# linnanwang/FastGen

Measured on AMD Instinct MI355X. Metric: images/sec at 4-step distilled (DMD2) sampling, higher is better.
Workload: dtype fp32 (tensors, accumulate) with split-bf16 x3 MFMA conv products; 1 GPU; EDM CIFAR-10 32x32 SongUNet (55.7M params) DMD2 4-step 'sde' sampling, batch=512 per GPU; global_batch=512, sample_steps=4, parallelism=replicas x1 (no data-path collective), graph=True

## Files before the change

### fastgen_amd/csrc/common.h

```cpp
#pragma once
#include <hip/hip_runtime.h>
#include <stdint.h>

typedef __attribute__((ext_vector_type(8))) __bf16 bf16x8;
typedef __attribute__((ext_vector_type(4))) __bf16 bf16x4;
typedef __attribute__((ext_vector_type(16))) float f32x16;
typedef __attribute__((ext_vector_type(4))) float f32x4;
typedef __attribute__((ext_vector_type(2))) float f32x2;

#define FG_WAVE 64

inline int fg_device_slot() {
    int dev = -1;
    return (hipGetDevice(&dev) == hipSuccess && dev >= 0 && dev < 16) ? dev : -1;
}

template <typename T>
struct DT;
template <>
struct DT<__bf16> {
    typedef __bf16 ST;
    typedef __bf16 WT;
    static constexpr int KC = 64;
    static constexpr int WPARTS = 1;
    static constexpr int FRAG_BYTES = 16;
    static constexpr bool FAST = true;
};
template <>
struct DT<float> {
    typedef float ST;
    typedef float WT;
    static constexpr int KC = 32;
    static constexpr int WPARTS = 1;
    static constexpr int FRAG_BYTES = 32;
    static constexpr bool FAST = false;
};
struct bf16x3 {};
template <>
struct DT<bf16x3> {
    typedef float ST;
    typedef __bf16 WT;
    static constexpr int KC = 32;
    static constexpr int WPARTS = 2;
    static constexpr int FRAG_BYTES = 16;
    static constexpr bool FAST = true;
};

template <typename T>
struct Frag8;
template <>
struct Frag8<__bf16> {
    bf16x8 v;
};
template <>
struct Frag8<float> {
    f32x4 lo, hi;
};
template <>
struct Frag8<bf16x3> {
    bf16x8 hi, lo;
};

__device__ __forceinline__ void mma16(f32x16& acc, const Frag8<__bf16>& a, const Frag8<__bf16>& b) {
    acc = __builtin_amdgcn_mfma_f32_32x32x16_bf16(a.v, b.v, acc, 0, 0, 0);
}
__device__ __forceinline__ void mma16(f32x16& acc, const Frag8<float>& a, const Frag8<float>& b) {
    acc = __builtin_amdgcn_mfma_f32_32x32x2f32(a.lo[0], b.lo[0], acc, 0, 0, 0);
    acc = __builtin_amdgcn_mfma_f32_32x32x2f32(a.lo[1], b.lo[1], acc, 0, 0, 0);
    acc = __builtin_amdgcn_mfma_f32_32x32x2f32(a.lo[2], b.lo[2], acc, 0, 0, 0);
    acc = __builtin_amdgcn_mfma_f32_32x32x2f32(a.lo[3], b.lo[3], acc, 0, 0, 0);
    acc = __builtin_amdgcn_mfma_f32_32x32x2f32(a.hi[0], b.hi[0], acc, 0, 0, 0);
    acc = __builtin_amdgcn_mfma_f32_32x32x2f32(a.hi[1], b.hi[1], acc, 0, 0, 0);
    acc = __builtin_amdgcn_mfma_f32_32x32x2f32(a.hi[2], b.hi[2], acc, 0, 0, 0);
    acc = __builtin_amdgcn_mfma_f32_32x32x2f32(a.hi[3], b.hi[3], acc, 0, 0, 0);
}

__device__ __forceinline__ void mma16(f32x16& acc, const Frag8<bf16x3>& a, const Frag8<bf16x3>& b) {
    acc = __builtin_amdgcn_mfma_f32_32x32x16_bf16(a.lo, b.hi, acc, 0, 0, 0);
    acc = __builtin_amdgcn_mfma_f32_32x32x16_bf16(a.hi, b.lo, acc, 0, 0, 0);
    acc = __builtin_amdgcn_mfma_f32_32x32x16_bf16(a.hi, b.hi, acc, 0, 0, 0);
}
__device__ __forceinline__ void split8(const float (&x)[8], bf16x8& hi, bf16x8& lo) {
#pragma unroll
    for (int j = 0; j < 8; ++j) {
        hi[j] = (__bf16)x[j];
        lo[j] = (__bf16)(x[j] - (float)hi[j]);
    }
}

typedef __attribute__((ext_vector_type(4))) unsigned fg_u32x4;
__device__ __forceinline__ __amdgpu_buffer_rsrc_t make_rsrc(const void* base) {
    return __builtin_amdgcn_make_buffer_rsrc(const_cast<void*>(base), 0, 0x7fffffff, 0x00020000);
}
__device__ __forceinline__ float fp8_wave_max(float v) {
#pragma unroll
    for (int o = 32; o > 0; o >>= 1) v = fmaxf(v, __shfl_xor(v, o));
    return v;
}
__device__ __forceinline__ float fp8_row_inv(float amax) { return amax == 0.f ? 1.0f : 448.0f / amax; }
__device__ __forceinline__ float fp8_row_scale(float amax) { return amax == 0.f ? 1.0f : amax / 448.0f; }
__device__ __forceinline__ unsigned fp8_pack4(f32x4 v, float inv) {
    float q[4];
#pragma unroll
    for (int e = 0; e < 4; ++e) q[e] = __builtin_amdgcn_fmed3f(v[e] * inv, -448.0f, 448.0f);
    int r = __builtin_amdgcn_cvt_pk_fp8_f32(q[0], q[1], 0, false);
    r = __builtin_amdgcn_cvt_pk_fp8_f32(q[2], q[3], r, true);
    return (unsigned)r;
}
__device__ __forceinline__ Frag8<__bf16> load_frag(const __bf16* p) {
    Frag8<__bf16> f;
    f.v = *reinterpret_cast<const bf16x8*>(p);
    return f;
}
__device__ __forceinline__ Frag8<float> load_frag(const float* p) {
    Frag8<float> f;
    f.lo = *reinterpret_cast<const f32x4*>(p);
    f.hi = *reinterpret_cast<const f32x4*>(p + 4);
    return f;
}
__device__ __forceinline__ void load_frag_rsrc(Frag8<__bf16>& f, __amdgpu_buffer_rsrc_t r, int lane_elems, int elem_off) {
    f.v = __builtin_bit_cast(bf16x8, __builtin_amdgcn_raw_buffer_load_b128(r, lane_elems * 2, elem_off * 2, 0));
}
__device__ __forceinline__ void load_frag_rsrc(Frag8<float>& f, __amdgpu_buffer_rsrc_t r, int lane_elems, int elem_off) {
    f.lo = __builtin_bit_cast(f32x4, __builtin_amdgcn_raw_buffer_load_b128(r, lane_elems * 4, elem_off * 4, 0));
    f.hi = __builtin_bit_cast(f32x4, __builtin_amdgcn_raw_buffer_load_b128(r, lane_elems * 4 + 16, elem_off * 4, 0));
}
__device__ __forceinline__ void load_frag_rsrc(Frag8<bf16x3>& f, __amdgpu_buffer_rsrc_t r, int lane_elems, int elem_off) {
    f.hi = __builtin_bit_cast(bf16x8, __builtin_amdgcn_raw_buffer_load_b128(r, lane_elems * 2, elem_off * 2, 0));
    f.lo = __builtin_bit_cast(bf16x8, __builtin_amdgcn_raw_buffer_load_b128(r, lane_elems * 2, elem_off * 2 + 1024, 0));
}
template <typename T>
__device__ __forceinline__ Frag8<T> load_wfrag(const typename DT<T>::WT* p) {
    return load_frag(p);
}
template <>
__device__ __forceinline__ Frag8<bf16x3> load_wfrag<bf16x3>(const __bf16* p) {
    Frag8<bf16x3> f;
    f.hi = *reinterpret_cast<const bf16x8*>(p);
    f.lo = *reinterpret_cast<const bf16x8*>(p + 512);
    return f;
}
template <typename T>
__device__ __forceinline__ Frag8<T> lds_read_a(const char* p, int kk);
template <>
__device__ __forceinline__ Frag8<__bf16> lds_read_a<__bf16>(const char* p, int kk) {
    Frag8<__bf16> f;
    f.v = *reinterpret_cast<const bf16x8*>(p + kk * 32);
    return f;
}
template <>
__device__ __forceinline__ Frag8<float> lds_read_a<float>(const char* p, int kk) {
    Frag8<float> f;
    f.lo = *reinterpret_cast<const f32x4*>(p + kk * 64);
    f.hi = *reinterpret_cast<const f32x4*>(p + kk * 64 + 16);
    return f;
}
template <>
__device__ __forceinline__ Frag8<bf16x3> lds_read_a<bf16x3>(const char* p, int kk) {
    Frag8<bf16x3> f;
    f.hi = *reinterpret_cast<const bf16x8*>(p + kk * 32);
    f.lo = *reinterpret_cast<const bf16x8*>(p + 64 + kk * 32);
    return f;
}
template <typename T>
__device__ __forceinline__ void lds_store_a(char* p, const float (&x)[8]);
__device__ __forceinline__ void store_frag(__bf16* p, const float (&x)[8]);
__device__ __forceinline__ void store_frag(float* p, const float (&x)[8]);
template <>
__device__ __forceinline__ void lds_store_a<__bf16>(char* p, const float (&x)[8]) { store_frag(reinterpret_cast<__bf16*>(p), x); }
template <>
__device__ __forceinline__ void lds_store_a<float>(char* p, const float (&x)[8]) { store_frag(reinterpret_cast<float*>(p), x); }
template <>
__device__ __forceinline__ void lds_store_a<bf16x3>(char* p, const float (&x)[8]) {
    bf16x8 hi, lo;
    split8(x, hi, lo);
    *reinterpret_cast<bf16x8*>(p) = hi;
    *reinterpret_cast<bf16x8*>(p + 64) = lo;
}
__device__ __forceinline__ void store_frag(__bf16* p, const float (&x)[8]) {
    bf16x8 v;
#pragma unroll
    for (int j = 0; j < 8; ++j) v[j] = (__bf16)x[j];
    *reinterpret_cast<bf16x8*>(p) = v;
}
__device__ __forceinline__ void store_frag(float* p, const float (&x)[8]) {
    *reinterpret_cast<f32x4*>(p) = f32x4{x[0], x[1], x[2], x[3]};
    *reinterpret_cast<f32x4*>(p + 4) = f32x4{x[4], x[5], x[6], x[7]};
}

__device__ __forceinline__ void widen8(const Frag8<__bf16>& f, float (&v)[8]) {
#pragma unroll
    for (int j = 0; j < 8; ++j) v[j] = (float)f.v[j];
}
__device__ __forceinline__ void widen8(const Frag8<float>& f, float (&v)[8]) {
    v[0] = f.lo[0]; v[1] = f.lo[1]; v[2] = f.lo[2]; v[3] = f.lo[3];
    v[4] = f.hi[0]; v[5] = f.hi[1]; v[6] = f.hi[2]; v[7] = f.hi[3];
}

__device__ __forceinline__ f32x4 load4(const float* p) { return *reinterpret_cast<const f32x4*>(p); }
__device__ __forceinline__ f32x4 load4(const __bf16* p) {
    const bf16x4 q = *reinterpret_cast<const bf16x4*>(p);
    return f32x4{(float)q[0], (float)q[1], (float)q[2], (float)q[3]};
}
__device__ __forceinline__ f32x4 store4(float* p, f32x4 v) {
    *reinterpret_cast<f32x4*>(p) = v;
    return v;
}
__device__ __forceinline__ f32x4 store4(__bf16* p, f32x4 v) {
    const bf16x4 q = {(__bf16)v[0], (__bf16)v[1], (__bf16)v[2], (__bf16)v[3]};
    *reinterpret_cast<bf16x4*>(p) = q;
    return f32x4{(float)q[0], (float)q[1], (float)q[2], (float)q[3]};
}

__device__ __forceinline__ f32x4 store4_split(__bf16* p, size_t lo_off, f32x4 v) {
    bf16x4 hi, lo;
#pragma unroll
    for (int j = 0; j < 4; ++j) {
        hi[j] = (__bf16)v[j];
        lo[j] = (__bf16)(v[j] - (float)hi[j]);
    }
    *reinterpret_cast<bf16x4*>(p) = hi;
    *reinterpret_cast<bf16x4*>(p + lo_off) = lo;
    return v;
}

template <typename T> struct Raw4;
template <> struct Raw4<float> { typedef f32x4 type; };
template <> struct Raw4<__bf16> { typedef bf16x4 type; };
__device__ __forceinline__ f32x4 raw_load4(const float* p) { return *reinterpret_cast<const f32x4*>(p); }
__device__ __forceinline__ bf16x4 raw_load4(const __bf16* p) { return *reinterpret_cast<const bf16x4*>(p); }
__device__ __forceinline__ f32x4 widen4(f32x4 v) { return v; }
__device__ __forceinline__ f32x4 widen4(bf16x4 q) { return f32x4{(float)q[0], (float)q[1], (float)q[2], (float)q[3]}; }

template <bool FAST>
__device__ __forceinline__ float silu_f(float x) {
    if (FAST) {
        float e = __builtin_amdgcn_exp2f(-1.44269504088896341f * x);
        return x * __builtin_amdgcn_rcpf(1.0f + e);
    } else {
        return x / (1.0f + expf(-x));
    }
}

__device__ __forceinline__ constexpr int acc_row(int i, int h) { return (i & 3) + 8 * (i >> 2) + 4 * h; }
```

### fastgen_amd/csrc/conv_ws3.hip

```cpp
#include "common.h"
#include "conv.h"

namespace {

constexpr int X3_NTHR = 768;
constexpr int X3_KC = 32;
constexpr int X3_PA = 16;
constexpr int X3_PLANE = 3072;
constexpr int X3_ABUF = 8 * X3_PLANE;
constexpr int X3_RING = 4;
constexpr int X3_HOFF = 128 * 512;
constexpr int X3_LDS = X3_HOFF + X3_RING * X3_ABUF;
constexpr int X3_TAPB = 2048;

template <int LOGW>
struct X3Geom {
    static constexpr int W = 1 << LOGW;
    static constexpr int TW = 16, TH = 8;
    static constexpr int IPT = LOGW == 3 ? 2 : 1;
    static constexpr int TCOLS = LOGW == 3 ? 1 : W / TW;
    static constexpr int TPI = LOGW == 3 ? 1 : (W / TH) * TCOLS;
    static constexpr int HW_ = LOGW == 3 ? 2 * W + 3 : TW + 2, HH_ = TH + 2;
    static constexpr int HALO_PIX = HW_ * HH_;
    static constexpr int RS = HW_ * X3_PA;
    static_assert(HALO_PIX * X3_PA <= X3_PLANE && HALO_PIX <= 192, "one halo plane; three producer passes of 64 pixels");
};

__device__ __forceinline__ void x3_barrier() {
    asm volatile("s_waitcnt lgkmcnt(0)\n\ts_barrier" ::: "memory");
}

struct X3Frag {
    bf16x8 hi, lo;
};

template <int RES, int LOGW, int PRO>
__global__ __launch_bounds__(X3_NTHR) void conv3_x3ws_kernel(const ConvArgs a, const int ntiles) {
    using G = X3Geom<LOGW>;
    constexpr bool SUB = RES == RES_SUBPIX;
    constexpr int NTAP = SUB ? 4 : 9;
    constexpr int RN = SUB ? 4 : 3;
    constexpr int NQ = 4 * NTAP;
    constexpr int X3_STEPB = NTAP * X3_TAPB;
    extern __shared__ __attribute__((aligned(16))) char smem[];
    char* const hbuf = smem;
    char* const ring = smem + X3_HOFF;

    const int tid = threadIdx.x;
    const int lane = tid & 63;
    const int wave = __builtin_amdgcn_readfirstlane(tid >> 6);
    const int Cin = a.C1 + a.C2;
    const int nchunk = Cin / X3_KC;
    const int G8 = (int)gridDim.x >> 3;
    const int wg = ((gridDim.x & 7) == 0) ? ((int)blockIdx.x & 7) * G8 + ((int)blockIdx.x >> 3) : (int)blockIdx.x;
    const int gstride = (int)gridDim.x;
    const int my_tiles = (ntiles - wg + gstride - 1) / gstride;
    const int S = my_tiles * nchunk;
    const int NSTEP = S + 3;
    const int H = SUB ? a.Hs : a.H;

    if (wave < 8) {
        const int grp = wave >> 2, wl = wave & 3;
        const int col = lane & 15, g4 = lane >> 4;
        const size_t wstride = (size_t)nchunk * NTAP * 1024;
        const __amdgpu_buffer_rsrc_t wrs = __builtin_amdgcn_make_buffer_rsrc(
            const_cast<__bf16*>(reinterpret_cast<const __bf16*>(a.wpack_ws) + (size_t)(grp * 8 + wl * 2) * wstride), 0, 0x7fffffff,
            0x00020000);
        const int wvoff = lane * 16;
        const int wsb = (int)(wstride * 2);
        const int wphb = SUB ? 16 * wsb : 0;
        int tcur = wg;
        auto load_w = [&](int byte_off) -> X3Frag {
            X3Frag f;
            f.hi = __builtin_bit_cast(bf16x8, __builtin_amdgcn_raw_buffer_load_b128(wrs, wvoff, byte_off, 0));
            f.lo = __builtin_bit_cast(bf16x8, __builtin_amdgcn_raw_buffer_load_b128(wrs, wvoff, byte_off + 1024, 0));
            return f;
        };
        X3Frag wq[RN][2];
#pragma unroll
        for (int j = 0; j < RN; ++j)
#pragma unroll
            for (int nt = 0; nt < 2; ++nt) wq[j][nt] = load_w((tcur & 3) * wphb + nt * wsb + (SUB ? j : 3 * j) * X3_TAPB);

        f32x4 acc[8][2];
#pragma unroll
        for (int m = 0; m < 8; ++m)
#pragma unroll
            for (int nt = 0; nt < 2; ++nt) acc[m][nt] = f32x4{0.f, 0.f, 0.f, 0.f};

        const int lane_off = g4 * X3_PLANE + (col + ((G::IPT == 2 && col >= 8) ? 1 : 0)) * X3_PA;
        const int dl0 = col * 512 + ((8 * wl + ((g4) ^ (col & 7))) << 4);
        const int dl1 = col * 512 + ((8 * wl + ((4 + g4) ^ (col & 7))) << 4);

        x3_barrier();
        int c = 0;
        for (int s = 0; s < NSTEP; ++s) {
            const int ls = s - 2 * grp;
            if (ls >= 0 && ls < S) {
                const char* abase = ring + (ls & 3) * X3_ABUF + lane_off + (SUB ? ((tcur >> 1) & 1) * G::RS + (tcur & 1) * X3_PA : 0);
                const int cn = (c + 1 == nchunk) ? 0 : c + 1;
                const int tnext = cn == 0 ? tcur + gstride : tcur;
                const int wcur = (tcur & 3) * wphb + c * X3_STEPB;
                const int wnxt = (ls + 1 < S) ? (tnext & 3) * wphb + cn * X3_STEPB : wcur;
                if constexpr (!SUB) {
                    const int trow = (tcur % G::TPI) / G::TCOLS;
                    const bool top = G::IPT == 2 || trow == 0;
                    const bool bot = G::IPT == 2 || trow == G::W / G::TH - 1;
                    auto read_row = [&](int i, X3Frag& xf) {
                        const int tx = i / G::HH_, h = i % G::HH_;
                        if ((h == 0 && top) || (h == G::HH_ - 1 && bot)) return;
                        xf.hi = *reinterpret_cast<const bf16x8*>(abase + h * G::RS + tx * X3_PA);
                        xf.lo = *reinterpret_cast<const bf16x8*>(abase + h * G::RS + tx * X3_PA + 4 * X3_PLANE);
                    };
                    auto mma_row = [&](int i, const X3Frag& xf) {
                        const int tx = i / G::HH_, h = i % G::HH_;
                        const bool live = !((h == 0 && top) || (h == G::HH_ - 1 && bot));
#pragma unroll
                        for (int ty = 0; ty < 3; ++ty) {
                            const int m = h - ty;
                            if (m < 0 || m >= G::TH) continue;
                            if (live) {
#pragma unroll
                                for (int term = 0; term < 3; ++term)
#pragma unroll
                                    for (int nt = 0; nt < 2; ++nt)
                                        acc[m][nt] = __builtin_amdgcn_mfma_f32_16x16x32_bf16(term == 1 ? wq[ty][nt].lo : wq[ty][nt].hi,
                                                                                             term == 0 ? xf.lo : xf.hi, acc[m][nt], 0, 0, 0);
                            }
                            if (m != G::TH - 1) continue;
                            const int pn = (tx < 2 ? wcur + (3 * ty + tx + 1) * X3_TAPB : wnxt + 3 * ty * X3_TAPB);
#pragma unroll
                            for (int nt = 0; nt < 2; ++nt) wq[ty][nt] = load_w(pn + nt * wsb);
                        }
                    };
                    X3Frag xr[2];
                    read_row(0, xr[0]);
#pragma unroll
                    for (int i = 0; i < 3 * G::HH_; ++i) {
                        if (i + 1 < 3 * G::HH_) read_row(i + 1, xr[(i + 1) & 1]);
                        __builtin_amdgcn_sched_barrier(0);
                        mma_row(i, xr[i & 1]);
                        __builtin_amdgcn_sched_barrier(0);
                    }
                } else {
                    auto read_x = [&](int q, X3Frag (&xf)[2]) {
                        const int tap = q >> 2, m0 = 2 * (q & 3);
                        const int off = ((tap >> 1) + m0) * G::RS + (tap & 1) * X3_PA;
#pragma unroll
                        for (int m = 0; m < 2; ++m) {
                            xf[m].hi = *reinterpret_cast<const bf16x8*>(abase + off + m * G::RS);
                            xf[m].lo = *reinterpret_cast<const bf16x8*>(abase + off + m * G::RS + 4 * X3_PLANE);
                        }
                    };
                    auto mma12 = [&](int q, const X3Frag (&xf)[2]) {
                        const int tap = q >> 2, m0 = 2 * (q & 3);
                        const X3Frag(&wf)[2] = wq[tap % RN];
#pragma unroll
                        for (int m = 0; m < 2; ++m)
#pragma unroll
                            for (int nt = 0; nt < 2; ++nt)
                                acc[m0 + m][nt] = __builtin_amdgcn_mfma_f32_16x16x32_bf16(wf[nt].hi, xf[m].lo, acc[m0 + m][nt], 0, 0, 0);
#pragma unroll
                        for (int m = 0; m < 2; ++m)
#pragma unroll
                            for (int nt = 0; nt < 2; ++nt)
                                acc[m0 + m][nt] = __builtin_amdgcn_mfma_f32_16x16x32_bf16(wf[nt].lo, xf[m].hi, acc[m0 + m][nt], 0, 0, 0);
#pragma unroll
                        for (int m = 0; m < 2; ++m)
#pragma unroll
                            for (int nt = 0; nt < 2; ++nt)
                                acc[m0 + m][nt] = __builtin_amdgcn_mfma_f32_16x16x32_bf16(wf[nt].hi, xf[m].hi, acc[m0 + m][nt], 0, 0, 0);
                        if ((q & 3) != 3) return;
                        const int pn = (tap + RN < NTAP) ? wcur + (tap + RN) * X3_TAPB : wnxt + (tap + RN - NTAP) * X3_TAPB;
#pragma unroll
                        for (int nt = 0; nt < 2; ++nt) wq[tap % RN][nt] = load_w(pn + nt * wsb);
                    };
                    X3Frag x0[2], x1[2];
                    read_x(0, x0);
#pragma unroll
                    for (int q = 0; q < NQ; q += 2) {
                        read_x(q + 1, x1);
                        __builtin_amdgcn_sched_barrier(0);
                        mma12(q, x0);
                        __builtin_amdgcn_sched_barrier(0);
                        if (q + 2 < NQ) read_x(q + 2, x0);
                        __builtin_amdgcn_sched_barrier(0);
                        mma12(q + 1, x1);
                        __builtin_amdgcn_sched_barrier(0);
                    }
                }
                if (c + 1 == nchunk) {
#pragma unroll
                    for (int m = 0; m < 8; ++m) {
                        *reinterpret_cast<f32x4*>(hbuf + m * 8192 + dl0) = acc[m][0];
                        *reinterpret_cast<f32x4*>(hbuf + m * 8192 + dl1) = acc[m][1];
                        acc[m][0] = f32x4{0.f, 0.f, 0.f, 0.f};
                        acc[m][1] = f32x4{0.f, 0.f, 0.f, 0.f};
                    }
                }
                c = cn;
                tcur = tnext;
            }
            x3_barrier();
        }
        return;
    }

    const int ptid = tid - 512;
    const int pw = wave - 8;
    const int oct = ptid & 3;
    const float* src1 = reinterpret_cast<const float*>(a.src1);
    const float* src2 = reinterpret_cast<const float*>(a.src2);
    int hdy[3], hdx[3], hlds[3];
    bool third;
    const int pslot = ptid >> 2;
    const int pimg = (G::IPT == 2 && pslot >= 30) ? 1 : 0;
#pragma unroll
    for (int i = 0; i < 3; ++i) {
        int hy, hx;
        if (G::IPT == 2) {
            const int l = pimg ? min(pslot - 30 + 34 * i, 99) : pslot + 30 * i;
            hy = pimg ? l / 10 : l / 9;
            hx = pimg ? 9 + (l - hy * 10) : l - hy * 9;
            third = pimg ? pslot - 30 + 68 < 100 : true;
        } else {
            const int hq = min(pslot + 64 * i, G::HALO_PIX - 1);
            hy = hq / G::HW_;
            hx = hq - hy * G::HW_;
            third = pslot + 128 < G::HALO_PIX;
        }
        hdy[i] = hy - 1;
        hdx[i] = hx - 1 - pimg * (G::W + 1);
        hlds[i] = oct * X3_PLANE + hy * G::RS + hx * X3_PA;
    }

    auto tile_coord = [&](int t, int& n, int& slot, int& row0, int& col0) {
        if (SUB) t >>= 2;
        n = t * G::IPT / G::TPI;
        slot = t - n * G::TPI / G::IPT;
        row0 = (slot / G::TCOLS) * G::TH;
        col0 = (slot % G::TCOLS) * G::TW;
    };

    struct Staged {
        f32x4 raw[3][2];
        float2 ab[8];
    };
    unsigned off1[3], off2[3];
    bool valid[3];
    const float2* abn = a.ab;
    auto tile_setup = [&](int t) __attribute__((always_inline)) {
        int n, slot, row0, col0;
        tile_coord(t, n, slot, row0, col0);
        bool in_batch = true;
        if (G::IPT == 2) {
            n += pimg;
            in_batch = n < a.B;
            n = min(n, a.B - 1);
        }
#pragma unroll
        for (int i = 0; i < 3; ++i) {
            const int y = row0 + hdy[i], x = col0 + hdx[i];
            valid[i] = (y >= 0) && (y < H) && (x >= 0) && (x < G::W) && (i < 2 || third) && in_batch;
            const int yc = min(max(y, 0), H - 1), xc = min(max(x, 0), G::W - 1);
            const int sy = (RES == RES_UP) ? (yc >> 1) : yc, sx = (RES == RES_UP) ? (xc >> 1) : xc;
            const unsigned pix = (unsigned)((n * a.Hs + sy) * a.Ws + sx);
            off1[i] = (pix * (unsigned)a.C1 + oct * 8) * 4u;
            off2[i] = (pix * (unsigned)a.C2 + oct * 8) * 4u;
        }
        abn = a.ab + (size_t)n * Cin;
    };
    auto stage_load = [&](Staged& st, int t, int c32) __attribute__((always_inline)) {
        if (c32 == 0) tile_setup(t);
        const bool first = c32 * X3_KC < a.C1;
        const char* base = first ? reinterpret_cast<const char*>(src1) + c32 * (X3_KC * 4)
                                 : reinterpret_cast<const char*>(src2) + (c32 * X3_KC - a.C1) * 4;
#pragma unroll
        for (int i = 0; i < 3; ++i) {
            const char* p = base + (first ? off1[i] : off2[i]);
            st.raw[i][0] = *reinterpret_cast<const f32x4*>(p);
            st.raw[i][1] = *reinterpret_cast<const f32x4*>(p + 16);
        }
        if (PRO == PRO_NONE) return;
        const float2* p = abn + c32 * X3_KC + oct * 8;
#pragma unroll
        for (int j = 0; j < 8; j += 2) {
            const f32x4 q = *reinterpret_cast<const f32x4*>(p + j);
            st.ab[j] = make_float2(q[0], q[1]);
            st.ab[j + 1] = make_float2(q[2], q[3]);
        }
    };
    auto stage_store = [&](const Staged& st, char* abuf) __attribute__((always_inline)) {
#pragma unroll
        for (int i = 0; i < 3; ++i) {
            float v[8];
#pragma unroll
            for (int j = 0; j < 8; ++j) {
                v[j] = st.raw[i][j >> 2][j & 3];
                if (PRO != PRO_NONE) v[j] = silu_f<true>(fmaf(v[j], st.ab[j].x, st.ab[j].y));
            }
            bf16x8 hi, lo;
            split8(v, hi, lo);
            typedef __attribute__((ext_vector_type(4))) unsigned u32x4;
            u32x4 wh = __builtin_bit_cast(u32x4, hi), wl_ = __builtin_bit_cast(u32x4, lo);
#pragma unroll
            for (int j = 0; j < 4; ++j) {
                wh[j] = valid[i] ? wh[j] : 0u;
                wl_[j] = valid[i] ? wl_[j] : 0u;
            }
            if (i < 2 || third) {
                *reinterpret_cast<u32x4*>(abuf + hlds[i]) = wh;
                *reinterpret_cast<u32x4*>(abuf + hlds[i] + 4 * X3_PLANE) = wl_;
            }
        }
    };

    const int chq = lane & 31, psub = lane >> 5;
    float* const out = reinterpret_cast<float*>(a.out);
    const float* const resid = reinterpret_cast<const float*>(a.resid);
    const bool has_resid = __builtin_amdgcn_readfirstlane(resid != nullptr);
    auto retire_half = [&](int t, int half) __attribute__((always_inline)) {
        int n, slot, row0, col0;
        tile_coord(t, n, slot, row0, col0);
        const int co = half * 128 + chq * 4;
        const int nimg = G::IPT == 2 ? min(2, a.B - n) : 1;
        f32x4 radd[G::IPT];
#pragma unroll
        for (int k = 0; k < G::IPT; ++k) {
            radd[k] = f32x4{0.f, 0.f, 0.f, 0.f};
            if (a.bias) radd[k] = *reinterpret_cast<const f32x4*>(a.bias + co);
            const int nk = G::IPT == 2 ? min(n + k, a.B - 1) : n;
            if (a.temb) radd[k] += *reinterpret_cast<const f32x4*>(a.temb + (size_t)nk * a.temb_stride + co);
            radd[k] *= a.scale;
        }
        constexpr int OW = SUB ? 2 * G::W : G::W, OST = SUB ? 2 : 1;
        const int ph = t & 3;
        const size_t tb = SUB ? (((size_t)n * (2 * H) + 2 * row0 + (ph >> 1)) * OW + 2 * col0 + (ph & 1)) * 256 + co
                              : (((size_t)n * H + row0) * G::W + col0) * 256 + co;
        const int rs = (SUB || G::IPT == 2) ? 0 : a.rshift;
        const size_t rtb = (SUB || G::IPT == 2) ? tb : (((size_t)n * (H >> rs) + (row0 >> rs)) * (G::W >> rs) + (col0 >> rs)) * 256 + co;
        float ssum[G::IPT] = {}, ssq[G::IPT] = {};
#pragma unroll 1
        for (int grp8 = 0; grp8 < 2; ++grp8) {
            f32x4 rr[8], dv[8];
            unsigned go[8];
#pragma unroll
            for (int j = 0; j < 8; ++j) {
                const int px = pw * 32 + 2 * (grp8 * 8 + j) + psub;
                unsigned rgo;
                if (G::IPT == 2) {
                    go[j] = (unsigned)((((j >> 2) * OW + OST * (px >> 4)) * OW + OST * (px & 7)) * 256);
                    rgo = go[j];
                } else {
                    go[j] = (unsigned)((OST * (px >> 4) * OW + OST * (px & 15)) * 256);
                    rgo = SUB ? go[j] : (unsigned)((((px >> 4) >> rs) * (G::W >> rs) + ((px & 15) >> rs)) * 256);
                }
                rr[j] = f32x4{0.f, 0.f, 0.f, 0.f};
                if (has_resid && (G::IPT == 1 || (j >> 2) < nimg)) rr[j] = *reinterpret_cast<const f32x4*>(resid + rtb + rgo);
                dv[j] = *reinterpret_cast<const f32x4*>(hbuf + px * 512 + ((chq ^ (px & 7)) << 4));
            }
#pragma unroll
            for (int j = 0; j < 8; ++j) {
                const int k = G::IPT == 2 ? j >> 2 : 0;
                if (G::IPT == 2 && k >= nimg) continue;
                f32x4 v;
#pragma unroll
                for (int e = 0; e < 4; ++e) v[e] = fmaf(dv[j][e], a.scale, radd[k][e]);
                if (has_resid) {
#pragma unroll
                    for (int e = 0; e < 4; ++e) v[e] = fmaf(rr[j][e], a.scale, v[e]);
                }
                *reinterpret_cast<f32x4*>(out + tb + go[j]) = v;
                ssum[k] += (v[0] + v[1]) + (v[2] + v[3]);
                ssq[k] += (v[0] * v[0] + v[1] * v[1]) + (v[2] * v[2] + v[3] * v[3]);
            }
        }
#pragma unroll
        for (int k = 0; k < G::IPT; ++k) {
            ssum[k] += __shfl_xor(ssum[k], 32);
            ssq[k] += __shfl_xor(ssq[k], 32);
            const size_t sl = SUB ? ((size_t)(n + k) * G::TPI + slot) * 4 + ph : (size_t)(n + k) * G::TPI + slot;
            if (a.stats && psub == 0 && k < nimg) a.stats[(sl * 4 + pw) * 64 + half * 32 + chq] = make_float2(ssum[k], ssq[k]);
        }
    };

    auto advance = [&](int& t, int& cc) {
        if (++cc == nchunk) {
            cc = 0;
            t += gstride;
        }
    };
    Staged st;
    int t1 = wg, c1 = 0;
    stage_load(st, t1, c1);
    stage_store(st, ring);
    advance(t1, c1);
    x3_barrier();
    int sa = 0;
    for (int s = 0; s < NSTEP; ++s) {
        const bool more = s + 1 < S;
        if (more) stage_load(st, t1, c1);
        if (sa == 0 && s >= nchunk && s <= S) retire_half(wg + (s / nchunk - 1) * gstride, 0);
        if (sa == 2 % nchunk && s - 2 >= nchunk && s - 2 <= S && (s - 2) % nchunk == 0) retire_half(wg + ((s - 2) / nchunk - 1) * gstride, 1);
        if (more) {
            stage_store(st, ring + ((s + 1) & 3) * X3_ABUF);
            advance(t1, c1);
        }
        if (++sa == nchunk) sa = 0;
        x3_barrier();
    }
}

__global__ void pack_conv_weights_x3ws_kernel(const float* __restrict__ w, __bf16* __restrict__ out, int cout, int cin) {
    const size_t total = (size_t)cout * cin * 9;
    const int nstep = cin / X3_KC;
    for (size_t idx = (size_t)blockIdx.x * blockDim.x + threadIdx.x; idx < total; idx += (size_t)gridDim.x * blockDim.x) {
        size_t t = idx;
        const int j = t % 8; t /= 8;
        const int lane = t % 64; t /= 64;
        const int tap = t % 9; t /= 9;
        const int step = t % nstep; t /= nstep;
        const int n16 = (int)t;
        const int co = n16 * 16 + (lane & 15);
        const int ci = step * X3_KC + 8 * (lane >> 4) + j;
        const float v = w[((size_t)co * cin + ci) * 9 + tap];
        const __bf16 hi = (__bf16)v;
        const size_t o = (idx / 512) * 1024 + (idx % 512);
        out[o] = hi;
        out[o + 512] = (__bf16)(v - (float)hi);
    }
}

__global__ void pack_conv_weights_x3sub_kernel(const float* __restrict__ w, __bf16* __restrict__ out, int cout, int cin) {
    const size_t total = (size_t)16 * cout * cin;
    const int nstep = cin / X3_KC, ng = cout / 16;
    for (size_t idx = (size_t)blockIdx.x * blockDim.x + threadIdx.x; idx < total; idx += (size_t)gridDim.x * blockDim.x) {
        size_t t = idx;
        const int j = t % 8; t /= 8;
        const int lane = t % 64; t /= 64;
        const int tap = t % 4; t /= 4;
        const int step = t % nstep; t /= nstep;
        const int n16 = t % ng; t /= ng;
        const int py = (int)t >> 1, px = (int)t & 1, ty = tap >> 1, tx = tap & 1;
        const int co = n16 * 16 + (lane & 15);
        const int ci = step * X3_KC + 8 * (lane >> 4) + j;
        const int ky0 = py ? 2 * ty : ty, ky1 = py ? ty + 1 : 2 * ty;
        const int kx0 = px ? 2 * tx : tx, kx1 = px ? tx + 1 : 2 * tx;
        const float* wp = w + ((size_t)co * cin + ci) * 9;
        float v = 0.f;
        for (int ky = ky0; ky <= ky1; ++ky)
            for (int kx = kx0; kx <= kx1; ++kx) v += wp[ky * 3 + kx];
        const __bf16 hi = (__bf16)v;
        const size_t o = (idx / 512) * 1024 + (idx % 512);
        out[o] = hi;
        out[o + 512] = (__bf16)(v - (float)hi);
    }
}

int g_x3_cus[16] = {};

template <int RES, int LOGW, int PRO>
int launch_x3_one(const ConvArgs& a, hipStream_t stream, bool prepare_only) {
    using G = X3Geom<LOGW>;
    auto kern = conv3_x3ws_kernel<RES, LOGW, PRO>;
    int dev = 0;
    if (hipGetDevice(&dev) != hipSuccess || dev < 0 || dev >= 16) return (int)hipErrorInvalidDevice;
    static bool attr_done[16] = {};
    if (!attr_done[dev]) {
        hipError_t e = hipFuncSetAttribute(reinterpret_cast<const void*>(kern), hipFuncAttributeMaxDynamicSharedMemorySize, X3_LDS);
        if (e != hipSuccess) return (int)e;
        attr_done[dev] = true;
    }
    if (!g_x3_cus[dev]) {
        int n = 0;
        if (hipDeviceGetAttribute(&n, hipDeviceAttributeMultiprocessorCount, dev) != hipSuccess || n <= 0) return (int)hipErrorUnknown;
        g_x3_cus[dev] = n;
    }
    if (prepare_only) return 0;
    const int ntiles = (a.B * G::TPI + G::IPT - 1) / G::IPT * (RES == RES_SUBPIX ? 4 : 1);
    const int grid = ntiles < g_x3_cus[dev] ? ntiles : g_x3_cus[dev];
    hipLaunchKernelGGL(kern, dim3(grid), dim3(X3_NTHR), X3_LDS, stream, a, ntiles);
    return (int)hipGetLastError();
}

}

int conv_x3ws_stat_slots(int W, int res) {
    if (res == RES_SUBPIX) return (W == 32 ? X3Geom<4>::TPI : X3Geom<3>::TPI) * 16;
    return (W == 32 ? X3Geom<5>::TPI : W == 16 ? X3Geom<4>::TPI : X3Geom<3>::TPI) * 4;
}

bool conv_x3ws_shape_ok(int cout, int cin, int res) {
    return cout == 256 && (res == 32 || res == 16 || res == 8) && (cin % X3_KC) == 0 && cin / X3_KC >= 4;
}

bool conv_x3ws_supported(int ks, int pro, int res, int outmode, const ConvArgs& a) {
    const int cin = a.C1 + a.C2;
    const size_t src_bytes = (size_t)a.B * a.Hs * a.Ws * (size_t)(a.C1 > a.C2 ? a.C1 : a.C2) * 4;
    if (src_bytes >= (1ull << 32)) return false;
    if (res == RES_SUBPIX)
        return ks == 3 && outmode == OUT_NHWC && pro == PRO_GN_SILU && a.ab && a.H == a.W && a.Hs == a.Ws && a.H == 2 * a.Hs && (a.Ws == 16 || a.Ws == 8) &&
               conv_x3ws_shape_ok(a.Cout, cin, a.Ws) && (a.C1 % X3_KC) == 0 && a.wpack_ws && !a.rshift;
    if (ks != 3 || outmode != OUT_NHWC || a.H != a.W || !conv_x3ws_shape_ok(a.Cout, cin, a.W) || (a.C1 % X3_KC) || !a.wpack_ws) return false;
    if (a.W == 8 && res != RES_NONE) return false;
    if (a.rshift && (a.rshift != 1 || !a.resid || a.W == 8 || res != RES_NONE)) return false;
    if (pro == PRO_NONE) return res == RES_NONE && a.Hs == a.H && a.Ws == a.W;
    return pro == PRO_GN_SILU && (res == RES_NONE || res == RES_UP) && a.ab != nullptr;
}

int launch_conv_x3ws(int res, const ConvArgs& a, hipStream_t stream, bool prepare_only, int pro) {
    if (res == RES_SUBPIX) {
        if (pro != PRO_GN_SILU || (a.Ws != 16 && a.Ws != 8)) return (int)hipErrorInvalidValue;
        return a.Ws == 16 ? launch_x3_one<RES_SUBPIX, 4, PRO_GN_SILU>(a, stream, prepare_only) : launch_x3_one<RES_SUBPIX, 3, PRO_GN_SILU>(a, stream, prepare_only);
    }
    if (pro == PRO_NONE || a.W == 8) {
        if (res != RES_NONE) return (int)hipErrorInvalidValue;
        if (a.W == 8)
            return pro == PRO_NONE ? launch_x3_one<RES_NONE, 3, PRO_NONE>(a, stream, prepare_only)
                                   : launch_x3_one<RES_NONE, 3, PRO_GN_SILU>(a, stream, prepare_only);
        return a.W == 32 ? launch_x3_one<RES_NONE, 5, PRO_NONE>(a, stream, prepare_only) : launch_x3_one<RES_NONE, 4, PRO_NONE>(a, stream, prepare_only);
    }
    if (a.W == 32)
        return res == RES_UP ? launch_x3_one<RES_UP, 5, PRO_GN_SILU>(a, stream, prepare_only) : launch_x3_one<RES_NONE, 5, PRO_GN_SILU>(a, stream, prepare_only);
    return res == RES_UP ? launch_x3_one<RES_UP, 4, PRO_GN_SILU>(a, stream, prepare_only) : launch_x3_one<RES_NONE, 4, PRO_GN_SILU>(a, stream, prepare_only);
}

int launch_pack_conv_weights_x3ws(const float* w_oihw, void* wpack_ws, int cout, int cin, hipStream_t stream) {
    const size_t total = (size_t)cout * cin * 9;
    const int grid = (int)((total + 255) / 256 < 4096 ? (total + 255) / 256 : 4096);
    hipLaunchKernelGGL(pack_conv_weights_x3ws_kernel, dim3(grid), dim3(256), 0, stream, w_oihw, (__bf16*)wpack_ws, cout, cin);
    return (int)hipGetLastError();
}

int launch_pack_conv_weights_x3sub(const float* w_oihw, void* wpack_sub, int cout, int cin, hipStream_t stream) {
    const size_t total = (size_t)16 * cout * cin;
    const int grid = (int)((total + 255) / 256 < 4096 ? (total + 255) / 256 : 4096);
    hipLaunchKernelGGL(pack_conv_weights_x3sub_kernel, dim3(grid), dim3(256), 0, stream, w_oihw, (__bf16*)wpack_sub, cout, cin);
    return (int)hipGetLastError();
}
```

Measured before the change: 2974 img/s.

## Streamline x3ws conv staging stores and epilogue with buffer ops and precomputed offsets

The producer's bf16 hi/lo split now uses packed pair conversions and writes to LDS through inline ds_write_b128 with immediate offsets, storing zeros only on invalid halo pixels. The epilogue switches to raw buffer loads and stores using 32-bit offsets and per-lane offsets precomputed once outside the loop. It also specialises the residual path at compile time and merges the two retire_half conditions into one. The aim is to cut VALU address arithmetic and conversion cost in the producer and epilogue. In exchange it adds a 4 GiB output-size guard and depends on hand-written asm offsets being correct.

After: 2992 img/s (median of 6 runs). Within noise of the previous version (+0.6%).

```diff
diff --git a/fastgen_amd/csrc/common.h b/fastgen_amd/csrc/common.h
--- a/fastgen_amd/csrc/common.h
+++ b/fastgen_amd/csrc/common.h
@@ -89,6 +89,17 @@
 }
 
 typedef __attribute__((ext_vector_type(4))) unsigned fg_u32x4;
+__device__ __forceinline__ void split8_pairs(const float (&x)[8], fg_u32x4& hi, fg_u32x4& lo) {
+    typedef __attribute__((ext_vector_type(2))) __bf16 bf16x2;
+#pragma unroll
+    for (int p = 0; p < 4; ++p) {
+        const unsigned h = __builtin_bit_cast(unsigned, __builtin_convertvector(f32x2{x[2 * p], x[2 * p + 1]}, bf16x2));
+        const float h0 = __builtin_bit_cast(float, h << 16), h1 = __builtin_bit_cast(float, h & 0xffff0000u);
+        hi[p] = h;
+        lo[p] = __builtin_bit_cast(unsigned, __builtin_convertvector(f32x2{x[2 * p] - h0, x[2 * p + 1] - h1}, bf16x2));
+    }
+}
+
 __device__ __forceinline__ __amdgpu_buffer_rsrc_t make_rsrc(const void* base) {
     return __builtin_amdgcn_make_buffer_rsrc(const_cast<void*>(base), 0, 0x7fffffff, 0x00020000);
 }
diff --git a/fastgen_amd/csrc/conv_ws3.hip b/fastgen_amd/csrc/conv_ws3.hip
--- a/fastgen_amd/csrc/conv_ws3.hip
+++ b/fastgen_amd/csrc/conv_ws3.hip
@@ -1,3 +1,5 @@
+#include <type_traits>
+
 #include "common.h"
 #include "conv.h"
 
@@ -28,6 +30,11 @@
 
 __device__ __forceinline__ void x3_barrier() {
     asm volatile("s_waitcnt lgkmcnt(0)\n\ts_barrier" ::: "memory");
+}
+
+template <int OFF>
+__device__ __forceinline__ void x3_lds_store(unsigned addr, fg_u32x4 q) {
+    asm volatile("ds_write_b128 %0, %1 offset:%2" ::"v"(addr), "v"(q), "i"(OFF) : "memory");
 }
 
 struct X3Frag {
@@ -246,6 +253,9 @@
         f32x4 raw[3][2];
         float2 ab[8];
     };
+    fg_u32x4 zq = {0u, 0u, 0u, 0u};
+    asm volatile("" : "+v"(zq));
+    const unsigned ring_lds = (unsigned)(uintptr_t)(__attribute__((address_space(3))) char*)ring;
     unsigned off1[3], off2[3];
     bool valid[3];
     const float2* abn = a.ab;
@@ -290,7 +300,7 @@
             st.ab[j + 1] = make_float2(q[2], q[3]);
         }
     };
-    auto stage_store = [&](const Staged& st, char* abuf) __attribute__((always_inline)) {
+    auto stage_store = [&](const Staged& st, unsigned abuf) __attribute__((always_inline)) {
 #pragma unroll
         for (int i = 0; i < 3; ++i) {
             float v[8];
@@ -299,18 +309,15 @@
                 v[j] = st.raw[i][j >> 2][j & 3];
                 if (PRO != PRO_NONE) v[j] = silu_f<true>(fmaf(v[j], st.ab[j].x, st.ab[j].y));
             }
-            bf16x8 hi, lo;
-            split8(v, hi, lo);
-            typedef __attribute__((ext_vector_type(4))) unsigned u32x4;
-            u32x4 wh = __builtin_bit_cast(u32x4, hi), wl_ = __builtin_bit_cast(u32x4, lo);
-#pragma unroll
-            for (int j = 0; j < 4; ++j) {
-                wh[j] = valid[i] ? wh[j] : 0u;
-                wl_[j] = valid[i] ? wl_[j] : 0u;
-            }
-            if (i < 2 || third) {
-                *reinterpret_cast<u32x4*>(abuf + hlds[i]) = wh;
-                *reinterpret_cast<u32x4*>(abuf + hlds[i] + 4 * X3_PLANE) = wl_;
+            fg_u32x4 wh, wl_;
+            split8_pairs(v, wh, wl_);
+            const unsigned la = abuf + hlds[i];
+            if (valid[i]) {
+                x3_lds_store<0>(la, wh);
+                x3_lds_store<4 * X3_PLANE>(la, wl_);
+            } else if (i < 2 || third) {
+                x3_lds_store<0>(la, zq);
+                x3_lds_store<4 * X3_PLANE>(la, zq);
             }
         }
     };
@@ -319,6 +326,19 @@
     float* const out = reinterpret_cast<float*>(a.out);
     const float* const resid = reinterpret_cast<const float*>(a.resid);
     const bool has_resid = __builtin_amdgcn_readfirstlane(resid != nullptr);
+    const unsigned out_bytes = (unsigned)a.B * a.H * a.W * 256u * 4u;
+    const __amdgpu_buffer_rsrc_t ors = __builtin_amdgcn_make_buffer_rsrc(out, 0, (int)out_bytes, 0x00020000);
+    const __amdgpu_buffer_rsrc_t rrs = __builtin_amdgcn_make_buffer_rsrc(const_cast<float*>(resid), 0, (int)(out_bytes >> (2 * a.rshift)), 0x00020000);
+    constexpr int OW = SUB ? 2 * G::W : G::W, OST = SUB ? 2 : 1;
+    const int rs = (SUB || G::IPT == 2) ? 0 : a.rshift;
+    const unsigned lgo = (unsigned)((OST * psub * 256 + chq * 4) * 4);
+    const unsigned lrgo = (unsigned)(((psub >> rs) * 256 + chq * 4) * 4);
+    unsigned lhx[4];
+#pragma unroll
+    for (int q = 0; q < 4; ++q) lhx[q] = (unsigned)(pw * 16384 + psub * 512 + ((chq ^ (2 * q + psub)) << 4));
+    auto pass_off = [](int j) constexpr { return G::IPT == 2 ? ((j >> 2) * OW * OW + OST * 2 * (j & 3)) * 256 : OST * 2 * j * 256; };
+    int ngrp8 = 2;
+    asm volatile("" : "+s"(ngrp8));
     auto retire_half = [&](int t, int half) __attribute__((always_inline)) {
         int n, slot, row0, col0;
         tile_coord(t, n, slot, row0, col0);
@@ -333,48 +353,49 @@
             if (a.temb) radd[k] += *reinterpret_cast<const f32x4*>(a.temb + (size_t)nk * a.temb_stride + co);
             radd[k] *= a.scale;
         }
-        constexpr int OW = SUB ? 2 * G::W : G::W, OST = SUB ? 2 : 1;
         const int ph = t & 3;
-        const size_t tb = SUB ? (((size_t)n * (2 * H) + 2 * row0 + (ph >> 1)) * OW + 2 * col0 + (ph & 1)) * 256 + co
-                              : (((size_t)n * H + row0) * G::W + col0) * 256 + co;
-        const int rs = (SUB || G::IPT == 2) ? 0 : a.rshift;
-        const size_t rtb = (SUB || G::IPT == 2) ? tb : (((size_t)n * (H >> rs) + (row0 >> rs)) * (G::W >> rs) + (col0 >> rs)) * 256 + co;
+        const unsigned tb = SUB ? (unsigned)(((n * (2 * H) + 2 * row0 + (ph >> 1)) * OW + 2 * col0 + (ph & 1)) * 256 + half * 128)
+                                : (unsigned)(((n * H + row0) * G::W + col0) * 256 + half * 128);
+        const unsigned rtb = (SUB || G::IPT == 2) ? tb : (unsigned)(((n * (H >> rs) + (row0 >> rs)) * (G::W >> rs) + (col0 >> rs)) * 256 + half * 128);
         float ssum[G::IPT] = {}, ssq[G::IPT] = {};
+        auto passes = [&](auto with_resid) __attribute__((always_inline)) {
+            constexpr bool HR = decltype(with_resid)::value;
 #pragma unroll 1
-        for (int grp8 = 0; grp8 < 2; ++grp8) {
-            f32x4 rr[8], dv[8];
-            unsigned go[8];
-#pragma unroll
-            for (int j = 0; j < 8; ++j) {
-                const int px = pw * 32 + 2 * (grp8 * 8 + j) + psub;
-                unsigned rgo;
-                if (G::IPT == 2) {
-                    go[j] = (unsigned)((((j >> 2) * OW + OST * (px >> 4)) * OW + OST * (px & 7)) * 256);
-                    rgo = go[j];
-                } else {
-                    go[j] = (unsigned)((OST * (px >> 4) * OW + OST * (px & 15)) * 256);
-                    rgo = SUB ? go[j] : (unsigned)((((px >> 4) >> rs) * (G::W >> rs) + ((px & 15) >> rs)) * 256);
+            for (int grp8 = 0; grp8 < ngrp8; ++grp8) {
+                const int prow = 2 * pw + grp8;
+                const unsigned ob = (tb + (unsigned)(OST * prow * OW * 256)) * 4;
+                const unsigned rb = (SUB || G::IPT == 2) ? ob : (rtb + (unsigned)((prow >> rs) * (G::W >> rs) * 256)) * 4;
+                const unsigned hb = (unsigned)(grp8 * 8192);
+                f32x4 rr[8], dv[8];
+#pragma unroll
+                for (int j = 0; j < 8; ++j) {
+                    if (HR && (G::IPT == 1 || (j >> 2) < nimg)) {
+                        const unsigned rbj = (SUB || G::IPT == 2) ? rb + pass_off(j) * 4 : rb + ((2 * j) >> rs) * 1024;
+                        rr[j] = __builtin_bit_cast(f32x4, __builtin_amdgcn_raw_buffer_load_b128(rrs, (SUB || G::IPT == 2) ? lgo : lrgo, rbj, 0));
+                    }
+                    dv[j] = *reinterpret_cast<const f32x4*>(hbuf + (lhx[j & 3] + hb) + j * 1024);
                 }
-                rr[j] = f32x4{0.f, 0.f, 0.f, 0.f};
-                if (has_resid && (G::IPT == 1 || (j >> 2) < nimg)) rr[j] = *reinterpret_cast<const f32x4*>(resid + rtb + rgo);
-                dv[j] = *reinterpret_cast<const f32x4*>(hbuf + px * 512 + ((chq ^ (px & 7)) << 4));
+#pragma unroll
+                for (int j = 0; j < 8; ++j) {
+                    const int k = G::IPT == 2 ? j >> 2 : 0;
+                    if (G::IPT == 2 && k >= nimg) continue;
+                    f32x4 v;
+#pragma unroll
+                    for (int e = 0; e < 4; ++e) v[e] = fmaf(dv[j][e], a.scale, radd[k][e]);
+                    if (HR) {
+#pragma unroll
+                        for (int e = 0; e < 4; ++e) v[e] = fmaf(rr[j][e], a.scale, v[e]);
+                    }
+                    __builtin_amdgcn_raw_buffer_store_b128(__builtin_bit_cast(fg_u32x4, v), ors, lgo, ob + pass_off(j) * 4, 0);
+                    ssum[k] += (v[0] + v[1]) + (v[2] + v[3]);
+                    ssq[k] += (v[0] * v[0] + v[1] * v[1]) + (v[2] * v[2] + v[3] * v[3]);
+                }
             }
-#pragma unroll
-            for (int j = 0; j < 8; ++j) {
-                const int k = G::IPT == 2 ? j >> 2 : 0;
-                if (G::IPT == 2 && k >= nimg) continue;
-                f32x4 v;
-#pragma unroll
-                for (int e = 0; e < 4; ++e) v[e] = fmaf(dv[j][e], a.scale, radd[k][e]);
-                if (has_resid) {
-#pragma unroll
-                    for (int e = 0; e < 4; ++e) v[e] = fmaf(rr[j][e], a.scale, v[e]);
-                }
-                *reinterpret_cast<f32x4*>(out + tb + go[j]) = v;
-                ssum[k] += (v[0] + v[1]) + (v[2] + v[3]);
-                ssq[k] += (v[0] * v[0] + v[1] * v[1]) + (v[2] * v[2] + v[3] * v[3]);
-            }
-        }
+        };
+        if (has_resid)
+            passes(std::true_type{});
+        else
+            passes(std::false_type{});
 #pragma unroll
         for (int k = 0; k < G::IPT; ++k) {
             ssum[k] += __shfl_xor(ssum[k], 32);
@@ -393,17 +414,17 @@
     Staged st;
     int t1 = wg, c1 = 0;
     stage_load(st, t1, c1);
-    stage_store(st, ring);
+    stage_store(st, ring_lds);
     advance(t1, c1);
     x3_barrier();
     int sa = 0;
     for (int s = 0; s < NSTEP; ++s) {
         const bool more = s + 1 < S;
         if (more) stage_load(st, t1, c1);
-        if (sa == 0 && s >= nchunk && s <= S) retire_half(wg + (s / nchunk - 1) * gstride, 0);
-        if (sa == 2 % nchunk && s - 2 >= nchunk && s - 2 <= S && (s - 2) % nchunk == 0) retire_half(wg + ((s - 2) / nchunk - 1) * gstride, 1);
+        const int half = sa == 0 ? 0 : 1, sr = s - 2 * half;
+        if ((sa == 0 || sa == 2) && sr >= nchunk && sr <= S) retire_half(wg + (sr / nchunk - 1) * gstride, half);
         if (more) {
-            stage_store(st, ring + ((s + 1) & 3) * X3_ABUF);
+            stage_store(st, ring_lds + ((s + 1) & 3) * X3_ABUF);
             advance(t1, c1);
         }
         if (++sa == nchunk) sa = 0;
@@ -498,6 +519,7 @@
     const int cin = a.C1 + a.C2;
     const size_t src_bytes = (size_t)a.B * a.Hs * a.Ws * (size_t)(a.C1 > a.C2 ? a.C1 : a.C2) * 4;
     if (src_bytes >= (1ull << 32)) return false;
+    if ((size_t)a.B * a.H * a.W * (size_t)a.Cout * 4 >= (1ull << 32)) return false;
     if (res == RES_SUBPIX)
         return ks == 3 && outmode == OUT_NHWC && pro == PRO_GN_SILU && a.ab && a.H == a.W && a.Hs == a.Ws && a.H == 2 * a.Hs && (a.Ws == 16 || a.Ws == 8) &&
                conv_x3ws_shape_ok(a.Cout, cin, a.Ws) && (a.C1 % X3_KC) == 0 && a.wpack_ws && !a.rshift;
```
